# distributed-lab/linea-stark-prover

Measured on AMD Instinct MI355X. Metric: prove time (s) + trace-rows/sec, 3x3 perm AIR @2^19; NTT HBM GB/s vs roofline, higher is better.
Workload: dtype fr253 (BLS12-377 Fr, 8x u32 Montgomery limbs); 1 GPU; 3x3 permutation AIR, 2^19 rows (w=8, q=4 quotient chunks, log_blowup 3, 33 queries, Poseidon2-w3 Merkle, FRI); log_n=19, width=8, fri_queries=33, parallelism=single-gpu

## Files before the change

linea_stark_prover_amd/csrc/capi.cpp:

```cpp
#include <hip/hip_runtime.h>

#include <algorithm>
#include <cstdlib>
#include <cstring>
#include <memory>
#include <thread>

#include "comm.hpp"
#include "prove_internal.hpp"

using namespace lsp;

namespace {
thread_local std::string g_err;

#ifdef LSP_DEBUG_BOUNDS
std::string bounds_fault_report() {
    int n = 0;
    if (hipGetDeviceCount(&n) != hipSuccess || n == 0) return "";
    (void)hipDeviceSynchronize();
    static const struct {
        const char* tu;
        unsigned (*reader)();
    } tus[] = {{"k_ntt.hip", bounds_fault_k_ntt},         {"k_hash.hip", bounds_fault_k_hash},
// ... 1573 lines not shown
            });
        } else {
            const Fr* b = d + (size_t)na * height;
            const Fr* af = b + (size_t)t->ntables * t->nbc * height;
            const Fr* bf = af + height;
            witness_block(ctx, trace, height, trace_w, col0, w, mem, [&](Fr* out, size_t stride) {
                witness_lookup_device(ctx, d, na, b, t->ntables, t->nbc, af, bf, height, al, de, out, stride);
            });
        }
        ctx->sync();
    });
}

int lsp_raw_trace_free(lsp_raw_trace* t) {
    delete t;
    return LSP_OK;
}

int lsp_calibrate_poseidon2(lsp_ctx* ctx, double* mperm_per_s) {
    return guarded(ctx, [&] {
        LSP_REQUIRE(ctx && mperm_per_s, LSP_E_ARG, "null");
        std::lock_guard<std::mutex> g(ctx->mu);
        need_gpu(ctx);
        const uint32_t iters = 4;
        Fr* out = ctx->fbuf("calib", (size_t)256 * 256 * 32);
        LSP_HIP(launch_calib_perm(out, (size_t)256 * 256 * 4, 1, ctx->rc29_dev, ctx->p2.L, ctx->stream));
        StreamTimer timer;
        double best = 0;
        for (size_t per_cu : {2, 4, 8, 16, 32}) {
            const size_t nth = (size_t)256 * 256 * per_cu;
            const float ms = timer.ms(ctx->stream, [&] {
                LSP_HIP(launch_calib_perm(out, nth, iters, ctx->rc29_dev, ctx->p2.L, ctx->stream));
            });
            best = std::max(best, (double)nth * iters / (ms * 1e-3) / 1e6);
        }
        *mperm_per_s = best;
    });
}

int lsp_calibrate_intt(lsp_ctx* ctx, uint32_t log_h, size_t w, double* gelem_per_s) {
    return guarded(ctx, [&] {
        LSP_REQUIRE(ctx && gelem_per_s, LSP_E_ARG, "null argument");
        LSP_REQUIRE(log_h >= 1 && log_h <= 26 && w >= 1 && w <= 1024 && (w << log_h) <= ((size_t)1 << 28), LSP_E_ARG,
                    "bad inverse-NTT probe shape (at most 2^28 elements)");
        std::lock_guard<std::mutex> g(ctx->mu);
        need_gpu(ctx);
        *gelem_per_s = calibrate_intt(ctx, log_h, w, 5, nullptr);
        ctx->release("calib_intt_");
    });
}

int lsp_gen_permutation_trace(uint64_t seed, uint32_t log_n, uint32_t ncols, const lsp_fr* alpha,
                              const lsp_fr* delta, int small_values, lsp_fr* rows) {
    return guarded(nullptr, [&] {
        LSP_REQUIRE(alpha && delta && rows && ncols >= 1 && log_n >= 1 && log_n <= 30, LSP_E_ARG,
                    "bad trace arguments");
        const size_t n = (size_t)1 << log_n, w = 2 * (size_t)ncols + 2;
        SplitMix64 g{seed ^ 0x5452414345ull};
        std::vector<Fr> a((size_t)ncols * n);
// ... 44 lines not shown
```

linea_stark_prover_amd/csrc/host.cpp:

```cpp
#include "host.hpp"

#include <algorithm>
#include <array>
#include <chrono>
#include <cstdlib>
#include <cstring>

#if defined(__linux__)
#include <sched.h>
#endif

#include "comm.hpp"

namespace lsp {

Fr host_generator() { return fr_from_u64(22); }

Fr host_inv_cached(const Fr& a) {
    static std::mutex mu;
    static std::map<std::array<uint32_t, 8>, Fr> cache;
    std::array<uint32_t, 8> k;
    for (int i = 0; i < 8; ++i) k[i] = a.v[i];
    {
        std::lock_guard<std::mutex> g(mu);
// ... 372 lines not shown
}

}

lsp_ctx::~lsp_ctx() {
    delete comm;
    if (device == LSP_HOST_ONLY || !stream) return;
    (void)hipSetDevice(device);
    (void)hipStreamSynchronize(stream);
    if (side_stream) (void)hipStreamSynchronize(side_stream);
    for (auto& kv : pool)
        if (kv.second.p) (void)hipFree(kv.second.p);
    for (auto& kv : hpool)
        if (kv.second.p) (void)hipHostFree(kv.second.p);
    for (auto& kv : stage_ev) (void)hipEventDestroy(kv.second);
    for (hipEvent_t e : event_pool) (void)hipEventDestroy(e);
    for (auto& t : pending_timings) {
        (void)hipEventDestroy(std::get<1>(t));
        (void)hipEventDestroy(std::get<2>(t));
    }
    if (ev_near) (void)hipEventDestroy(ev_near);
    if (ev_top) (void)hipEventDestroy(ev_top);
    if (ev_warm) (void)hipEventDestroy(ev_warm);
    if (side_stream) {
        (void)hipStreamSynchronize(side_stream);
        (void)hipEventDestroy(ev_wide);
        (void)hipEventDestroy(ev_side);
        (void)hipStreamDestroy(side_stream);
    }
    if (rc_dev) (void)hipFree(rc_dev);
    if (rc29_dev) (void)hipFree(rc29_dev);
    (void)hipStreamDestroy(stream);
}

void* lsp_ctx::buf(const std::string& name, size_t bytes) {
    Buf& b = pool[name];
    if (b.cap < bytes) {
        if (b.p) {
            LSP_HIP(hipStreamSynchronize(stream));
            LSP_HIP(hipFree(b.p));
            b.p = nullptr;
            b.cap = 0;
        }
        if (bytes) {
            hipError_t e = hipMalloc(&b.p, bytes);
            if (e != hipSuccess) {
// ... 102 lines not shown
```

linea_stark_prover_amd/csrc/host.hpp:

```cpp
#pragma once
#include <hip/hip_runtime.h>

#include <algorithm>
#include <atomic>
#include <condition_variable>
#include <functional>
#include <map>
#include <memory>
#include <mutex>
#include <thread>
#include <tuple>
#include <stdexcept>
#include <string>
#include <utility>
#include <vector>

#include "../../include/lsp.h"
#include "air_walk.hpp"
#include "fr.hpp"
#include "kernels.hpp"
#include "poseidon2.hpp"
#include "poseidon2_host64.hpp"

namespace lsp {
// ... 382 lines not shown
    int device = 0;
    lsp::Comm* comm = nullptr;
    std::unique_ptr<lsp::HostPool> pool_;
    size_t host_tree_top = 1024;
    hipStream_t stream = nullptr;
    lsp::P2Host p2;
    lsp::Fr* rc_dev = nullptr;
    lsp::F29* rc29_dev = nullptr;
    uint32_t log_blowup = 3, log_final_poly_len = 0, num_queries = 33, pow_bits = 0;
    size_t lds_per_block = 64 * 1024;
    int32_t public_degree = 1;
    lsp::TranscriptCfg transcript;
    std::string err;
    std::mutex mu;
    struct Buf {
        void* p = nullptr;
        size_t cap = 0;
    };
    std::map<std::string, Buf> pool;
    std::map<std::string, Buf> hpool;
    std::map<std::string, hipEvent_t> stage_ev;
    hipEvent_t ev_near = nullptr, ev_top = nullptr;
    hipEvent_t ev_warm = nullptr;
    hipStream_t side_stream = nullptr;
    hipEvent_t ev_wide = nullptr, ev_side = nullptr;
    hipStream_t side();
    std::vector<hipEvent_t> event_pool;
    bool phase_timing = true;
    std::vector<std::string> phase_only;
    std::map<std::string, const lsp::Fr*> tables;
    const lsp::Fr* table(const std::string& key, size_t n, const std::function<void(lsp::Fr*)>& fill,
                         const char* scratch = nullptr);
    struct TopUpload {
        void* dst;
        const void* src;
        size_t bytes;
    };
    bool defer_top_uploads = false;
    std::vector<TopUpload> top_uploads;
    std::map<uint32_t, std::vector<lsp::Fr>> fold_tw;
    size_t fri_host_tail = 2048;
    std::vector<std::pair<std::string, double>> timings;
    std::vector<std::tuple<std::string, hipEvent_t, hipEvent_t>> pending_timings;
    std::vector<std::string> spans;

    void* buf(const std::string& name, size_t bytes);
// ... 14 lines not shown
```

linea_stark_prover_amd/csrc/k_hash.hip:

```cpp
#include <cstdlib>

#include "k_common.hpp"
#include "kernels.hpp"
#include "p2_launch.hpp"
#include "poseidon2_f29.hpp"
#include "poseidon2_row.hpp"

namespace lsp {

#ifndef LSP_P2_ROWS_WPE
#define LSP_P2_ROWS_WPE 1
#endif

namespace {
template <uint32_t D>
__global__ __launch_bounds__(256) void k_permute(Fr* __restrict__ st, size_t n, const F29* __restrict__ rc,
                                                 uint32_t rf, uint32_t rp) {
    __shared__ uint4 qt[3 * F29_QTAB_N];
    f29_qtab_init(qt);
    __syncthreads();
    const size_t i = gtid();
    if (i >= n) return;
    F29 s0 = f29_from_fr(st[3 * i]), s1 = f29_from_fr(st[3 * i + 1]), s2 = f29_from_fr(st[3 * i + 2]);
    permute3_any<D, 1>(s0, s1, s2, rc, rf, rp, qt);
// ... 192 lines not shown

hipError_t launch_merkle_level(const Fr* src, Fr* dst, size_t nout, const F29* rc, P2Layout L, hipStream_t st) {
    if (!nout) return hipSuccess;
    if (!L.gen_lin && nout <= row_max()) {
        if (L.sbox_degree == 17)
            hipLaunchKernelGGL(k_merkle_level_row<17>, dim3((unsigned)nout), dim3(64), 0, st, src, dst, nout, rc,
                               L.rounds_f, L.rounds_p);
        else
            hipLaunchKernelGGL(k_merkle_level_row<11>, dim3((unsigned)nout), dim3(64), 0, st, src, dst, nout, rc,
                               L.rounds_f, L.rounds_p);
        return hipGetLastError();
    }
    const int lanes = lanes_for(nout);
    unsigned blocks, bs;
    state_grid(nout, lanes, blocks, bs);
    p2_dispatch(L, lanes, [&](auto d, auto ln) {
        hipLaunchKernelGGL((k_merkle_level<decltype(d)::value, decltype(ln)::value>), dim3(blocks), dim3(bs), 0, st,
                           src, dst, nout, rc, L.rounds_f, L.rounds_p);
    });
    return hipGetLastError();
}

hipError_t launch_merkle_levels(Fr* layers, size_t nleaves, size_t stop_len, const F29* rc, P2Layout L,
                                size_t* off_out, size_t* len_out, hipStream_t st) {
    size_t off = 0, len = nleaves;
    while (len > stop_len && len > 1) {
        hipError_t e = launch_merkle_level(layers + off, layers + off + len, len / 2, rc, L, st);
        if (e != hipSuccess) return e;
        off += len;
        len /= 2;
    }
    *off_out = off;
    *len_out = len;
    return hipSuccess;
}

hipError_t launch_merkle_tree(Fr* layers, size_t nleaves, const F29* rc, P2Layout L, hipStream_t st) {
    size_t off = 0, len = nleaves;
    while (len > 128) {
        const size_t nout = len / 2;
        hipError_t e = launch_merkle_level(layers + off, layers + off + len, nout, rc, L, st);
        if (e != hipSuccess) return e;
        off += len;
        len /= 2;
    }
    if (len > 1) {
        p2_dispatch(L, [&](auto d) {
            hipLaunchKernelGGL(k_merkle_top<decltype(d)::value>, dim3(1), dim3(256), 0, st, layers, off, (uint32_t)len,
                               rc, L.rounds_f, L.rounds_p);
        });
// ... 9 lines not shown
```

linea_stark_prover_amd/csrc/kernels.hpp:

```cpp
#pragma once
#include <hip/hip_runtime.h>
#include <stddef.h>
#include <stdint.h>

#include "fr.hpp"
#include "fr29.hpp"
#include "ntt_plan.hpp"
#include "poseidon2.hpp"

namespace lsp {

constexpr uint32_t COLMAP_PLAIN = 0xffu;
struct ColMap {
    uint32_t logb = COLMAP_PLAIN;
    uint32_t stride = 0, c0 = 0, cstep = 1, valid = 0xffffffffu;
    uint32_t bw = 0;
    static ColMap plain(uint32_t w) {
        ColMap m;
        m.stride = w;
        m.valid = w;
        return m;
    }
    static ColMap blocked(uint32_t logb, uint32_t bw) {
        ColMap m;
// ... 28 lines not shown
                             Fr* tabs, hipStream_t st);
hipError_t launch_powers(const Fr* tab, uint32_t L1, size_t n, Fr* out, hipStream_t st);

struct MatList {
    const Fr* ptr[8];
    uint32_t width[8];
    uint32_t n;
};
inline MatList one_mat(const Fr* p, uint32_t w) {
    MatList m{};
    m.ptr[0] = p;
    m.width[0] = w;
    m.n = 1;
    return m;
}
hipError_t launch_rc_to_f29(const Fr* rc, F29* rc29, uint32_t n, hipStream_t st);
hipError_t launch_permute(Fr* states, size_t n, const F29* rc29, P2Layout L, hipStream_t st);
hipError_t launch_hash_rows(const MatList& m, size_t nrows, Fr* out, const F29* rc29, P2Layout L, hipStream_t st);
hipError_t launch_merkle_level(const Fr* src, Fr* dst, size_t nout, const F29* rc29, P2Layout L, hipStream_t st);
hipError_t launch_grind(const Fr pre[3], uint32_t wlane, uint64_t base, uint64_t count, uint32_t bits, bool mont,
                        const F29* rc29, P2Layout L, unsigned long long* best, hipStream_t st);
hipError_t launch_merkle_tree(Fr* layers, size_t nleaves, const F29* rc29, P2Layout L, hipStream_t st);
hipError_t launch_merkle_levels(Fr* layers, size_t nleaves, size_t stop_len, const F29* rc29, P2Layout L,
                                size_t* off_out, size_t* len_out, hipStream_t st);

hipError_t launch_merkle_inject(const Fr* src, const Fr* inj, Fr* dst, size_t nout, const F29* rc29, P2Layout L,
                                hipStream_t st);

struct FoldSpec {
    const Fr* v;
    Fr* vout;
    Fr half, half_beta;
    const Fr* tab;
    uint32_t L1, logm;
    uint64_t i0;
    const Fr* add;
};
hipError_t launch_fold_hash(const FoldSpec& f, size_t nleaves, Fr* out, const F29* rc29, P2Layout L, hipStream_t st);
hipError_t launch_fri_fold(const FoldSpec& f, size_t m, hipStream_t st);

size_t batch_inverse_scratch(size_t n);
hipError_t launch_batch_inverse(const Fr* in, Fr* out, size_t n, hipStream_t st, Fr* scratch,
                                const Fr* inv_total = nullptr);
hipError_t launch_calib_mul(Fr* out, size_t nthreads, uint32_t iters, hipStream_t st);
hipError_t launch_calib_perm(Fr* out, size_t nthreads, uint32_t iters, const F29* rc, P2Layout L, hipStream_t st);
hipError_t launch_gather(const uint64_t* ptrs, Fr* out, size_t n, hipStream_t st);
hipError_t launch_assemble_chunks(const Fr* stage, uint32_t logGq, size_t Sq, Fr* out, hipStream_t st);
// ... 125 lines not shown
```

linea_stark_prover_amd/csrc/merkle.cpp:

```cpp
#include <hip/hip_runtime.h>

#include <algorithm>
#include <atomic>
#include <chrono>
#include <cstdio>
#include <cstdlib>

#include "comm.hpp"
#include "host.hpp"
#include "prove_internal.hpp"

namespace lsp {

struct TopTimes {
    bool on = std::getenv("LSP_TIME_TOPS") != nullptr;
    double sync_us = 0, levels_us = 0, first_us = 0;
    size_t n = 0;
    struct Rec { size_t height; double since_prev, launch, near, spin, levels; };
    std::vector<Rec> recs;
    host_clock::time_point last_exit{};
    ~TopTimes() {
        if (on && n) {
            std::fprintf(stderr, "[tree tops] %zu trees: wait-for-GPU %.1f us, host levels %.1f us (first level %.1f us) per tree\n",
                         n, sync_us / n, levels_us / n, first_us / n);
            const size_t k = recs.size() < 16 ? 0 : recs.size() - 16;
            for (size_t i = k; i < recs.size(); ++i)
                std::fprintf(stderr, "[tree] height %9zu  since-prev %7.1f  launch %6.1f  near %8.1f  spin %7.1f  levels %6.1f us\n",
                             recs[i].height, recs[i].since_prev, recs[i].launch, recs[i].near, recs[i].spin, recs[i].levels);
        }
    }
};
static TopTimes g_top_times;
bool time_tops() { return g_top_times.on; }

static std::atomic<int> g_active_proofs{0};
ActiveProof::ActiveProof() { g_active_proofs.fetch_add(1, std::memory_order_relaxed); }
ActiveProof::~ActiveProof() { g_active_proofs.fetch_sub(1, std::memory_order_relaxed); }
constexpr size_t SHARED_HOST_TREE_TOP = 256;

static void host_compress_level(lsp_ctx* ctx, const Fr* in, Fr* out, size_t half) {
    HostPool& pool = ctx->host_pool();
    if (half <= pool.size())
        pool.parallel_for(half, [&](size_t i) { out[i] = ctx->p2.compress(in[2 * i], in[2 * i + 1]); });
    else {
        const size_t blk = half >= 16 * pool.size() ? 16 : 8;
        pool.parallel_for((half + blk - 1) / blk, [&](size_t b) {
            ctx->p2.compress_range(in, out, blk * b, std::min(half, blk * b + blk));
        });
    }
}

// ... 38 lines not shown
    }
    size_t P = 1;
    while (2 * P <= pool.size() && first / (2 * P) >= 16) P *= 2;
    const size_t per = first / P;
    const uint32_t sl = log2_exact(per);
    auto task = [&](size_t p) {
        if (pairs) leaf_part(p * per, per);
        for (uint32_t j = 1; j <= sl; ++j) level_part(j, p * (per >> j), per >> j);
    };
    if (P > 1)
        pool.parallel_for(P, task);
    else
        task(0);
    if (t_first) *t_first = std::chrono::steady_clock::now();
    for (uint32_t j = sl + 1; j <= nl; ++j) level_part(j, 0, first >> j);
    return end;
}

static std::string top_buf_name(lsp_ctx* ctx) {
    return ctx->defer_top_uploads ? "merkle_top" + std::to_string(ctx->top_uploads.size()) : std::string("merkle_top");
}

void flush_top_uploads(lsp_ctx* ctx) {
    for (const auto& u : ctx->top_uploads)
        LSP_HIP(hipMemcpyAsync(u.dst, u.src, u.bytes, hipMemcpyHostToDevice, ctx->stream));
    ctx->top_uploads.clear();
}

DeferTopUploads::DeferTopUploads(lsp_ctx* c) : ctx(c) {
    ctx->top_uploads.clear();
    ctx->defer_top_uploads = std::getenv("LSP_NO_DEFER_TOPS") == nullptr;
}
DeferTopUploads::~DeferTopUploads() {
    ctx->defer_top_uploads = false;
    ctx->top_uploads.clear();
}

static bool zerocopy_top() {
    static const bool on = [] {
        const char* e = std::getenv("LSP_TOP_ZEROCOPY");
        return !(e && *e == '0');
    }();
    return on;
}

constexpr size_t WIDE_LEVEL_STOP = (size_t)1 << 16;

static size_t top_warm_nodes(const lsp_ctx* ctx) {
    if (const char* e = std::getenv("LSP_TOP_WARM")) return (size_t)std::strtoull(e, nullptr, 10);
    static const bool shared_host = [] {
        const char* e = std::getenv("LOCAL_WORLD_SIZE");
        return e && std::strtol(e, nullptr, 10) > 1;
    }();
    if (shared_host || ctx->comm || g_active_proofs.load(std::memory_order_relaxed) > 1) return 0;
    return (size_t)1 << 20;
}
constexpr unsigned TOP_WARM_SPIN_US = 5000;

static void spin_until(hipEvent_t ev) {
    hipError_t q;
    while ((q = hipEventQuery(ev)) == hipErrorNotReady) {
#if defined(__x86_64__)
        __builtin_ia32_pause();
#endif
    }
    LSP_HIP(q);
}

size_t host_tree_top(const lsp_ctx* ctx) {
    size_t top = ctx->host_tree_top;
    if (g_active_proofs.load(std::memory_order_relaxed) > 1) top = std::min(top, SHARED_HOST_TREE_TOP);
    return env_size("LSP_HOST_TREE_TOP", top);
}

Fr commit_device(lsp_ctx* ctx, const MatList& m, size_t height, Fr* layers, size_t top, const FoldSpec* fold,
                 const std::function<void(hipEvent_t)>* side) {
    hipStream_t st = ctx->stream;
    using clk = host_clock;
    const auto tt0 = clk::now();
    auto t_launched = tt0, t_near = tt0;
    HostPool& pool = ctx->host_pool();
    size_t off = 0, len = height;
    if (fold && height <= top && height > 1) {
        LSP_HIP(launch_fri_fold(*fold, 2 * height, st));
        fold = nullptr;
    }
    const bool leaves_on_host = height <= top && m.n == 1 && height > 1;
    bool gpu_level_on_host = false;
    Fr* host;
    if (leaves_on_host) {
        const size_t w = m.width[0];
        host = (Fr*)ctx->hbuf(top_buf_name(ctx), (TreeLayout{height}.size() + height * w) * sizeof(Fr));
        Fr* rows = host + TreeLayout{height}.size();
        LSP_HIP(hipMemcpyAsync(rows, m.ptr[0], height * w * sizeof(Fr), hipMemcpyDeviceToHost, st));
        if (side) {
            LSP_HIP(hipEventRecord(ctx->ev_wide, st));
            (*side)(ctx->ev_wide);
        }
        LSP_HIP(hipStreamSynchronize(st));
        pool.parallel_for((height + 7) / 8, [&](size_t b) {
            ctx->p2.hash_range(rows, w, host, 8 * b, std::min(height, 8 * b + 8));
        });
    } else {
        if (fold)
            LSP_HIP(launch_fold_hash(*fold, height, layers, ctx->rc29_dev, ctx->p2.L, st));
        else
            LSP_HIP(launch_hash_rows(m, height, layers, ctx->rc29_dev, ctx->p2.L, st));
        if (top == 0) {
            LSP_HIP(launch_merkle_tree(layers, height, ctx->rc29_dev, ctx->p2.L, st));
            if (side) {
                LSP_HIP(hipEventRecord(ctx->ev_wide, st));
                (*side)(ctx->ev_wide);
            }
            return d2h_fr(ctx, layers + TreeLayout{height}.root());
        }
        if (!ctx->ev_near) {
            LSP_HIP(hipEventCreateWithFlags(&ctx->ev_near, hipEventDisableTiming));
            LSP_HIP(hipEventCreateWithFlags(&ctx->ev_top, hipEventDisableTiming));
            LSP_HIP(hipEventCreateWithFlags(&ctx->ev_warm, hipEventDisableTiming));
        }
        const size_t warm = top_warm_nodes(ctx);
        struct Stop {
            size_t nodes;
            hipEvent_t ev;
        } stops[2];
        int nstops = 0;
        if (warm) stops[nstops++] = {std::max(4 * top, warm), ctx->ev_warm};
        if (side) stops[nstops++] = {std::max(4 * top, WIDE_LEVEL_STOP), ctx->ev_wide};
        if (nstops == 2 && stops[1].nodes > stops[0].nodes) std::swap(stops[0], stops[1]);
        size_t off1 = 0, len1 = height;
        auto levels_to = [&](size_t stop, hipEvent_t ev = nullptr) {
            size_t o = 0, l = len1;
            LSP_HIP(launch_merkle_levels(layers + off1, len1, stop, ctx->rc29_dev, ctx->p2.L, &o, &l, st));
            if (ev) LSP_HIP(hipEventRecord(ev, st));
            off1 += o;
            len1 = l;
        };
        for (int k = 0; k < nstops; ++k) levels_to(stops[k].nodes, stops[k].ev);
        levels_to(4 * top, ctx->ev_near);
        if (zerocopy_top()) levels_to(2 * top);
        if (zerocopy_top() && len1 > top) {
            off = off1;
            len = len1 / 2;
            host = (Fr*)ctx->hbuf(top_buf_name(ctx) + "c", TreeLayout{len}.size() * sizeof(Fr), hipHostMallocCoherent);
            LSP_HIP(launch_merkle_level(layers + off, host, len, ctx->rc29_dev, ctx->p2.L, st));
            off += len1;
            gpu_level_on_host = true;
        } else {
            if (!zerocopy_top()) levels_to(top);
            off = off1;
            len = len1;
            host = (Fr*)ctx->hbuf(top_buf_name(ctx), TreeLayout{len}.size() * sizeof(Fr));
            LSP_HIP(hipMemcpyAsync(host, layers + off, len * sizeof(Fr), hipMemcpyDeviceToHost, st));
        }
        LSP_HIP(hipEventRecord(ctx->ev_top, st));
        if (side) (*side)(ctx->ev_wide);
        t_launched = clk::now();
        resolve_timings(ctx);
        if (warm) {
            LSP_HIP(hipEventSynchronize(ctx->ev_warm));
            pool.wake(TOP_WARM_SPIN_US);
            spin_until(ctx->ev_near);
            t_near = clk::now();
        } else {
            LSP_HIP(hipEventSynchronize(ctx->ev_near));
            t_near = clk::now();
            pool.wake();
        }
        spin_until(ctx->ev_top);
    }
    const auto tt1 = clk::now();
    auto tt2 = tt1;
    const size_t first = len;
    const size_t end = host_levels(ctx, host, first, &tt2);
    if (g_top_times.on) {
        const auto tt3 = clk::now();
        g_top_times.n++;
        g_top_times.sync_us += us(tt0, tt1);
        g_top_times.levels_us += us(tt1, tt3);
        g_top_times.first_us += us(tt1, tt2);
        g_top_times.recs.push_back({height, g_top_times.last_exit == clk::time_point{} ? 0.0 : us(g_top_times.last_exit, tt0),
                                    us(tt0, t_launched), us(t_launched, t_near), us(t_near, tt1), us(tt1, tt3)});
        g_top_times.last_exit = clk::now();
    }
    const size_t skip = leaves_on_host || gpu_level_on_host ? 0 : first;
    if (end > skip) {
        if (ctx->defer_top_uploads)
            ctx->top_uploads.push_back({layers + off + skip, host + skip, (end - skip) * sizeof(Fr)});
        else
            LSP_HIP(hipMemcpyAsync(layers + off + skip, host + skip, (end - skip) * sizeof(Fr), hipMemcpyHostToDevice, st));
    }
    return host[end - 1];
}

Fr shard_root(lsp_ctx* ctx, Comm& comm, const Fr& local, std::vector<std::vector<Fr>>& top, const char* tag) {
    if (comm.size == 1) {
        top.assign(1, std::vector<Fr>(1, local));
        return local;
    }
    top.assign(1, comm.allgather_fr(ctx, &local, 1, tag));
    while (top.back().size() > 1) {
        const std::vector<Fr>& lo = top.back();
        std::vector<Fr> up(lo.size() / 2);
        for (size_t i = 0; i < up.size(); ++i) up[i] = ctx->p2.compress(lo[2 * i], lo[2 * i + 1]);
        top.push_back(std::move(up));
// ... 6 lines not shown
```

linea_stark_prover_amd/csrc/merkle_mixed.cpp:

```cpp
#include <hip/hip_runtime.h>

#include <algorithm>

#include "host.hpp"
#include "prove_internal.hpp"

namespace lsp {

std::vector<HeightClass> height_classes(const size_t* widths, const size_t* heights, size_t nmats) {
    LSP_REQUIRE(widths && heights && nmats >= 1, LSP_E_ARG, "a batch needs at least one matrix");
    std::vector<size_t> order(nmats);
    for (size_t k = 0; k < nmats; ++k) {
        LSP_REQUIRE(widths[k] >= 1 && widths[k] <= ((size_t)1 << 20), LSP_E_ARG, "matrix width outside [1, 2^20]");
        LSP_REQUIRE(heights[k] <= ((size_t)1 << 40), LSP_E_SIZE, "matrix height beyond 2^40");
        log2_exact(heights[k]);
        LSP_REQUIRE(heights[k] * widths[k] <= ((size_t)1 << 48), LSP_E_SIZE, "matrix beyond 2^48 elements");
        order[k] = k;
    }
    std::stable_sort(order.begin(), order.end(), [&](size_t a, size_t b) { return heights[a] > heights[b]; });
    std::vector<HeightClass> cls;
    for (size_t k : order) {
        if (cls.empty() || cls.back().height != heights[k]) cls.push_back({heights[k], {}});
        LSP_REQUIRE(cls.back().idx.size() < 8, LSP_E_ARG, "more than 8 matrices of one height");
        cls.back().idx.push_back(k);
    }
    return cls;
}
// ... 14 lines not shown
        (void)hipGetLastError();
        throw LspError(LSP_E_OOM, std::string("hipMalloc of ") + what + " failed");
    }
    return d;
}

std::unique_ptr<lsp_tree> new_tree(lsp_ctx* ctx, size_t leaves, size_t nmats, const size_t* heights,
                                   const size_t* widths, const lsp_fr* const* src, int mem) {
    auto t = std::make_unique<lsp_tree>(ctx, leaves);
    t->widths.assign(widths, widths + nmats);
    t->heights.assign(heights, heights + nmats);
    for (size_t k = 0; k < nmats; ++k) {
        const size_t n = heights[k] * widths[k];
        t->mats.push_back(dev_alloc_fr(n, "a tree's matrix"));
        if (src)
            LSP_HIP(hipMemcpyAsync(t->mats[k], src[k], n * sizeof(Fr),
                                   mem == LSP_MEM_DEVICE ? hipMemcpyDeviceToDevice : hipMemcpyHostToDevice,
                                   ctx->stream));
    }
    t->layers = dev_alloc_fr(TreeLayout{leaves}.size(), "a tree's layers");
    return t;
}

Fr commit_mixed_device(lsp_ctx* ctx, const std::vector<HeightClass>& cls, const Fr* const* mats, const size_t* widths,
                       Fr* layers) {
    hipStream_t st = ctx->stream;
    const TreeLayout lay{cls[0].height};
    for (const HeightClass& c : cls) {
        MatList m{};
        m.n = (uint32_t)c.idx.size();
        for (uint32_t j = 0; j < m.n; ++j) {
            m.ptr[j] = mats[c.idx[j]];
            m.width[j] = (uint32_t)widths[c.idx[j]];
        }
        LSP_HIP(launch_hash_rows(m, c.height, layers + lay.offset_of_len(c.height), ctx->rc29_dev, ctx->p2.L, st));
    }
    size_t off = 0, len = lay.leaves, next = 1;
    while (len > 1) {
        if (next == cls.size()) {
            LSP_HIP(launch_merkle_tree(layers + off, len, ctx->rc29_dev, ctx->p2.L, st));
            break;
        }
        const size_t nout = len / 2;
        Fr* dst = layers + off + len;
        if (cls[next].height == nout) {
            LSP_HIP(launch_merkle_inject(layers + off, dst, dst, nout, ctx->rc29_dev, ctx->p2.L, st));
            ++next;
        } else
            LSP_HIP(launch_merkle_level(layers + off, dst, nout, ctx->rc29_dev, ctx->p2.L, st));
        off += len;
        len = nout;
    }
    return d2h_fr(ctx, layers + lay.root());
}

bool verify_mixed_host(const lsp_ctx* ctx, const Fr& root, const std::vector<HeightClass>& cls, const size_t* widths,
                       size_t nmats, size_t index, const lsp_fr* rows, const lsp_fr* path) {
    std::vector<size_t> at(nmats + 1, 0);
    for (size_t k = 0; k < nmats; ++k) at[k + 1] = at[k] + widths[k];
    auto class_hash = [&](const HeightClass& c) {
// ... 18 lines not shown
```

linea_stark_prover_amd/csrc/p2_launch.hpp:

```cpp
#pragma once
#include <cstdlib>
#include <type_traits>

#include "k_common.hpp"
#include "poseidon2.hpp"
#include "poseidon2_f29.hpp"

namespace lsp {

inline size_t p2_env_size(const char* name, size_t dflt) {
    const char* e = std::getenv(name);
    return e ? (size_t)std::strtoull(e, nullptr, 10) : dflt;
}
inline size_t coop_max() {
    static const size_t v = p2_env_size("LSP_COOP_MAX", 16384);
    return v;
}
inline size_t pair_max() {
    static const size_t v = p2_env_size("LSP_PAIR_MAX", 32768);
    return v;
}
inline unsigned coop_bs() {
    static const unsigned v = (unsigned)p2_env_size("LSP_COOP_BS", 0);
    return v;
}
inline int lanes_for(size_t n) { return n <= coop_max() ? 4 : (n <= pair_max() ? 2 : 1); }

inline void state_grid(size_t n, int lanes, unsigned& blocks, unsigned& bs) {
    bs = lanes == 4 ? (coop_bs() ? coop_bs() : (4 * n >= 65536 ? 256u : 64u)) : 256u;
    blocks = nblocks((size_t)lanes * n, bs);
}

template <class F>
inline void p2_dispatch(const P2Layout& L, F&& f) {
    if (L.gen_lin) {
        if (L.sbox_degree == 17)
            f(std::integral_constant<uint32_t, 17u | P2_GEN>{});
        else
            f(std::integral_constant<uint32_t, 11u | P2_GEN>{});
    } else if (L.sbox_degree == 17)
        f(std::integral_constant<uint32_t, 17u>{});
    else
        f(std::integral_constant<uint32_t, 11u>{});
}
template <class F>
inline void p2_dispatch(const P2Layout& L, int lanes, F&& f) {
    p2_dispatch(L, [&](auto d) {
        if (lanes == 4)
            f(d, std::integral_constant<int, 4>{});
        else if (lanes == 2)
            f(d, std::integral_constant<int, 2>{});
        else
// ... 6 lines not shown
```

linea_stark_prover_amd/csrc/prove_internal.hpp:

```cpp
#pragma once
#include <chrono>
#include <cstdlib>
#include <functional>
#include <string>
#include <vector>

#include "host.hpp"

namespace lsp {
struct Comm;
bool time_tops();
using host_clock = std::chrono::steady_clock;
inline double us(host_clock::time_point a, host_clock::time_point b) {
    return std::chrono::duration<double, std::micro>(b - a).count();
}
inline size_t env_size(const char* name, size_t dflt) {
    const char* e = std::getenv(name);
    return e ? (size_t)std::strtoull(e, nullptr, 10) : dflt;
}
const Fr* pow_table(lsp_ctx* ctx, const Fr& base, uint32_t bits, uint32_t& L1);
Fr d2h_fr(lsp_ctx* ctx, const Fr* d);
struct LdeRequest {
    const Fr* src = nullptr;
    bool coeffs = false;
// ... 43 lines not shown
};
template <class Sibling, class AfterLevel>
Fr merkle_path_root(const P2Host& p2, Fr cur, size_t index, uint32_t levels, Sibling&& sibling,
                    AfterLevel&& after_level) {
    for (uint32_t l = 0; l < levels; ++l) {
        const Fr sib = sibling(l);
        cur = after_level(l + 1, ((index >> l) & 1) ? p2.compress(sib, cur) : p2.compress(cur, sib));
    }
    return cur;
}
inline Fr no_injection(uint32_t, const Fr& cur) { return cur; }
std::unique_ptr<lsp_tree> new_tree(lsp_ctx* ctx, size_t leaves, size_t nmats, const size_t* heights,
                                   const size_t* widths, const lsp_fr* const* src, int mem);
struct ActiveProof {
    ActiveProof();
    ~ActiveProof();
};
struct DeferTopUploads {
    lsp_ctx* ctx;
    explicit DeferTopUploads(lsp_ctx* c);
    ~DeferTopUploads();
};
void flush_top_uploads(lsp_ctx* ctx);
size_t host_levels(lsp_ctx* ctx, Fr* host, size_t first, host_clock::time_point* t_first = nullptr,
                   const Fr* pairs = nullptr);
Fr shard_root(lsp_ctx* ctx, Comm& comm, const Fr& local, std::vector<std::vector<Fr>>& top, const char* tag);
void lde_device(lsp_ctx* ctx, const Fr* d_in, size_t h, size_t w, uint32_t added_bits, const Fr* shifts_host,
                Fr* d_out);
void coset_dft_device(lsp_ctx* ctx, const Fr* d_coef, size_t h, size_t w, const Fr& shift, Fr* d_out);
void coset_idft_device(lsp_ctx* ctx, const Fr* d_evals, size_t h, size_t w, const Fr& shift, Fr* d_out);
void resolve_timings(lsp_ctx* ctx);
size_t host_tree_top(const lsp_ctx* ctx);
Fr commit_device(lsp_ctx* ctx, const MatList& m, size_t height, Fr* layers, size_t top, const FoldSpec* fold = nullptr,
                 const std::function<void(hipEvent_t)>* side = nullptr);
struct HeightClass {
    size_t height;
    std::vector<size_t> idx;
};
std::vector<HeightClass> height_classes(const size_t* widths, const size_t* heights, size_t nmats);
Fr commit_mixed_device(lsp_ctx* ctx, const std::vector<HeightClass>& cls, const Fr* const* mats, const size_t* widths,
                       Fr* layers);
bool verify_mixed_host(const lsp_ctx* ctx, const Fr& root, const std::vector<HeightClass>& cls, const size_t* widths,
                       size_t nmats, size_t index, const lsp_fr* rows, const lsp_fr* path);
uint64_t grind_device(lsp_ctx* ctx, Challenger& ch, uint32_t bits);
struct FriRound {
    const Fr* vec;
// ... 128 lines not shown
```

Baseline: 8.653 million trace-rows/s.

## Offload tail slice of large Merkle leaf hashing to host thread pool

For large commit trees (at least 2^21 leaves, single proof, zero-copy top), the last 1/32 to 1/128 of leaf rows is copied to the host on the side stream. There the CPU pool hashes and compresses that slice into the join level while the GPU hashes the remaining prefix. The slice size is picked from one-time calibrated GPU and host Poseidon2 permutation rates, and the host-computed layers are uploaded back into the device tree. The intent is to shave GPU hashing time by using idle CPU cores, at the cost of extra D2H/H2D traffic, a first-call calibration, and more synchronisation. Separately, the 4-lane cooperative block size now switches to 256 threads at a lower element count.

Result: faster. 8.740 million trace-rows/s, median of 6 (+1.0%).

```diff
diff --git a/linea_stark_prover_amd/csrc/capi.cpp b/linea_stark_prover_amd/csrc/capi.cpp
--- a/linea_stark_prover_amd/csrc/capi.cpp
+++ b/linea_stark_prover_amd/csrc/capi.cpp
@@ -1619,19 +1619,7 @@
         LSP_REQUIRE(ctx && mperm_per_s, LSP_E_ARG, "null");
         std::lock_guard<std::mutex> g(ctx->mu);
         need_gpu(ctx);
-        const uint32_t iters = 4;
-        Fr* out = ctx->fbuf("calib", (size_t)256 * 256 * 32);
-        LSP_HIP(launch_calib_perm(out, (size_t)256 * 256 * 4, 1, ctx->rc29_dev, ctx->p2.L, ctx->stream));
-        StreamTimer timer;
-        double best = 0;
-        for (size_t per_cu : {2, 4, 8, 16, 32}) {
-            const size_t nth = (size_t)256 * 256 * per_cu;
-            const float ms = timer.ms(ctx->stream, [&] {
-                LSP_HIP(launch_calib_perm(out, nth, iters, ctx->rc29_dev, ctx->p2.L, ctx->stream));
-            });
-            best = std::max(best, (double)nth * iters / (ms * 1e-3) / 1e6);
-        }
-        *mperm_per_s = best;
+        *mperm_per_s = calibrate_poseidon2(ctx);
     });
 }
 
diff --git a/linea_stark_prover_amd/csrc/host.cpp b/linea_stark_prover_amd/csrc/host.cpp
--- a/linea_stark_prover_amd/csrc/host.cpp
+++ b/linea_stark_prover_amd/csrc/host.cpp
@@ -418,6 +418,9 @@
     if (ev_near) (void)hipEventDestroy(ev_near);
     if (ev_top) (void)hipEventDestroy(ev_top);
     if (ev_warm) (void)hipEventDestroy(ev_warm);
+    if (ev_slice_in) (void)hipEventDestroy(ev_slice_in);
+    if (ev_slice) (void)hipEventDestroy(ev_slice);
+    if (ev_slice_up) (void)hipEventDestroy(ev_slice_up);
     if (side_stream) {
         (void)hipStreamSynchronize(side_stream);
         (void)hipEventDestroy(ev_wide);
diff --git a/linea_stark_prover_amd/csrc/host.hpp b/linea_stark_prover_amd/csrc/host.hpp
--- a/linea_stark_prover_amd/csrc/host.hpp
+++ b/linea_stark_prover_amd/csrc/host.hpp
@@ -428,6 +428,10 @@
     std::map<std::string, hipEvent_t> stage_ev;
     hipEvent_t ev_near = nullptr, ev_top = nullptr;
     hipEvent_t ev_warm = nullptr;
+    hipEvent_t ev_slice_in = nullptr, ev_slice = nullptr;
+    double slice_host_perm_s = 0, slice_gpu_perm_s = 0;
+    hipEvent_t ev_slice_up = nullptr;
+    bool slice_uploads_pending = false;
     hipStream_t side_stream = nullptr;
     hipEvent_t ev_wide = nullptr, ev_side = nullptr;
     hipStream_t side();
diff --git a/linea_stark_prover_amd/csrc/host_slice.hpp b/linea_stark_prover_amd/csrc/host_slice.hpp
--- /dev/null
+++ b/linea_stark_prover_amd/csrc/host_slice.hpp
@@ -0,0 +1,52 @@
+#pragma once
+#include <cstddef>
+#include <cstdint>
+
+namespace lsp {
+
+constexpr size_t HOST_SLICE_MIN_LEAVES = (size_t)1 << 21;
+constexpr double HOST_SLICE_MARGIN = 0.85;
+constexpr uint32_t HOST_SLICE_LOG_FRAC_FIRST = 5, HOST_SLICE_LOG_FRAC_LAST = 7;
+
+struct HostSliceIn {
+    size_t leaves = 0;
+    size_t perms_per_leaf = 1;
+    size_t join = 0;
+    double host_perm_s = 0;
+    double gpu_perm_s = 0;
+    bool shared = false;
+    int forced = -1;
+};
+
+struct HostSlice {
+    uint32_t log_frac = 0;
+    explicit operator bool() const { return log_frac != 0; }
+    size_t slice(size_t len) const { return log_frac ? len >> log_frac : 0; }
+    size_t prefix(size_t len) const { return len - slice(len); }
+};
+
+inline double slice_perms(size_t leaves, size_t perms_per_leaf, size_t roots) {
+    return (double)leaves * (double)perms_per_leaf + (double)(leaves - roots);
+}
+
+inline bool host_slice_fits(const HostSliceIn& in, uint32_t log_frac) {
+    if (log_frac == 0 || log_frac >= 8 * sizeof(size_t)) return false;
+    if (in.join == 0 || (in.join & (in.join - 1)) || in.leaves <= in.join || (in.leaves & (in.leaves - 1))) return false;
+    return (in.join >> log_frac) >= 1;
+}
+
+inline HostSlice plan_host_slice(const HostSliceIn& in) {
+    if (in.forced == 0) return {};
+    if (in.forced > 0) return host_slice_fits(in, (uint32_t)in.forced) ? HostSlice{(uint32_t)in.forced} : HostSlice{};
+    if (in.shared || in.leaves < HOST_SLICE_MIN_LEAVES || !(in.host_perm_s > 0) || !(in.gpu_perm_s > 0)) return {};
+    for (uint32_t lf = HOST_SLICE_LOG_FRAC_FIRST; lf <= HOST_SLICE_LOG_FRAC_LAST; ++lf) {
+        if (!host_slice_fits(in, lf)) break;
+        const HostSlice s{lf};
+        const double host_s = slice_perms(s.slice(in.leaves), in.perms_per_leaf, s.slice(in.join)) / in.host_perm_s;
+        const double gpu_s = slice_perms(s.prefix(in.leaves), in.perms_per_leaf, s.prefix(in.join)) / in.gpu_perm_s;
+        if (host_s <= HOST_SLICE_MARGIN * gpu_s) return s;
+    }
+    return {};
+}
+
+}
diff --git a/linea_stark_prover_amd/csrc/k_hash.hip b/linea_stark_prover_amd/csrc/k_hash.hip
--- a/linea_stark_prover_amd/csrc/k_hash.hip
+++ b/linea_stark_prover_amd/csrc/k_hash.hip
@@ -238,10 +238,11 @@
 }
 
 hipError_t launch_merkle_levels(Fr* layers, size_t nleaves, size_t stop_len, const F29* rc, P2Layout L,
-                                size_t* off_out, size_t* len_out, hipStream_t st) {
+                                size_t* off_out, size_t* len_out, hipStream_t st, uint32_t skip_log_frac) {
     size_t off = 0, len = nleaves;
     while (len > stop_len && len > 1) {
-        hipError_t e = launch_merkle_level(layers + off, layers + off + len, len / 2, rc, L, st);
+        const size_t nout = len / 2, skip = skip_log_frac ? nout >> skip_log_frac : 0;
+        hipError_t e = launch_merkle_level(layers + off, layers + off + len, nout - skip, rc, L, st);
         if (e != hipSuccess) return e;
         off += len;
         len /= 2;
diff --git a/linea_stark_prover_amd/csrc/kernels.hpp b/linea_stark_prover_amd/csrc/kernels.hpp
--- a/linea_stark_prover_amd/csrc/kernels.hpp
+++ b/linea_stark_prover_amd/csrc/kernels.hpp
@@ -74,7 +74,7 @@
                         const F29* rc29, P2Layout L, unsigned long long* best, hipStream_t st);
 hipError_t launch_merkle_tree(Fr* layers, size_t nleaves, const F29* rc29, P2Layout L, hipStream_t st);
 hipError_t launch_merkle_levels(Fr* layers, size_t nleaves, size_t stop_len, const F29* rc29, P2Layout L,
-                                size_t* off_out, size_t* len_out, hipStream_t st);
+                                size_t* off_out, size_t* len_out, hipStream_t st, uint32_t skip_log_frac = 0);
 
 hipError_t launch_merkle_inject(const Fr* src, const Fr* inj, Fr* dst, size_t nout, const F29* rc29, P2Layout L,
                                 hipStream_t st);
diff --git a/linea_stark_prover_amd/csrc/merkle.cpp b/linea_stark_prover_amd/csrc/merkle.cpp
--- a/linea_stark_prover_amd/csrc/merkle.cpp
+++ b/linea_stark_prover_amd/csrc/merkle.cpp
@@ -8,6 +8,7 @@
 
 #include "comm.hpp"
 #include "host.hpp"
+#include "host_slice.hpp"
 #include "prove_internal.hpp"
 
 namespace lsp {
@@ -16,7 +17,7 @@
     bool on = std::getenv("LSP_TIME_TOPS") != nullptr;
     double sync_us = 0, levels_us = 0, first_us = 0;
     size_t n = 0;
-    struct Rec { size_t height; double since_prev, launch, near, spin, levels; };
+    struct Rec { size_t height; double since_prev, launch, near, spin, levels, slice; };
     std::vector<Rec> recs;
     host_clock::time_point last_exit{};
     ~TopTimes() {
@@ -25,8 +26,8 @@
                          n, sync_us / n, levels_us / n, first_us / n);
             const size_t k = recs.size() < 16 ? 0 : recs.size() - 16;
             for (size_t i = k; i < recs.size(); ++i)
-                std::fprintf(stderr, "[tree] height %9zu  since-prev %7.1f  launch %6.1f  near %8.1f  spin %7.1f  levels %6.1f us\n",
-                             recs[i].height, recs[i].since_prev, recs[i].launch, recs[i].near, recs[i].spin, recs[i].levels);
+                std::fprintf(stderr, "[tree] height %9zu  since-prev %7.1f  launch %6.1f  near %8.1f  spin %7.1f  levels %6.1f  host slice %8.1f us\n",
+                             recs[i].height, recs[i].since_prev, recs[i].launch, recs[i].near, recs[i].spin, recs[i].levels, recs[i].slice);
         }
     }
 };
@@ -111,6 +112,10 @@
 }
 
 void flush_top_uploads(lsp_ctx* ctx) {
+    if (ctx->slice_uploads_pending) {
+        LSP_HIP(hipStreamWaitEvent(ctx->stream, ctx->ev_slice_up, 0));
+        ctx->slice_uploads_pending = false;
+    }
     for (const auto& u : ctx->top_uploads)
         LSP_HIP(hipMemcpyAsync(u.dst, u.src, u.bytes, hipMemcpyHostToDevice, ctx->stream));
     ctx->top_uploads.clear();
@@ -122,6 +127,7 @@
 }
 DeferTopUploads::~DeferTopUploads() {
     ctx->defer_top_uploads = false;
+    ctx->slice_uploads_pending = false;
     ctx->top_uploads.clear();
 }
 
@@ -135,13 +141,16 @@
 
 constexpr size_t WIDE_LEVEL_STOP = (size_t)1 << 16;
 
-static size_t top_warm_nodes(const lsp_ctx* ctx) {
-    if (const char* e = std::getenv("LSP_TOP_WARM")) return (size_t)std::strtoull(e, nullptr, 10);
-    static const bool shared_host = [] {
+static bool shared_host() {
+    static const bool v = [] {
         const char* e = std::getenv("LOCAL_WORLD_SIZE");
         return e && std::strtol(e, nullptr, 10) > 1;
     }();
-    if (shared_host || ctx->comm || g_active_proofs.load(std::memory_order_relaxed) > 1) return 0;
+    return v;
+}
+static size_t top_warm_nodes(const lsp_ctx* ctx) {
+    if (const char* e = std::getenv("LSP_TOP_WARM")) return (size_t)std::strtoull(e, nullptr, 10);
+    if (shared_host() || ctx->comm || g_active_proofs.load(std::memory_order_relaxed) > 1) return 0;
     return (size_t)1 << 20;
 }
 constexpr unsigned TOP_WARM_SPIN_US = 5000;
@@ -160,6 +169,159 @@
     size_t top = ctx->host_tree_top;
     if (g_active_proofs.load(std::memory_order_relaxed) > 1) top = std::min(top, SHARED_HOST_TREE_TOP);
     return env_size("LSP_HOST_TREE_TOP", top);
+}
+
+double calibrate_poseidon2(lsp_ctx* ctx) {
+    const uint32_t iters = 4;
+    Fr* out = ctx->fbuf("calib", (size_t)256 * 256 * 32);
+    LSP_HIP(launch_calib_perm(out, (size_t)256 * 256 * 4, 1, ctx->rc29_dev, ctx->p2.L, ctx->stream));
+    StreamTimer timer;
+    double best = 0;
+    for (size_t per_cu : {2, 4, 8, 16, 32}) {
+        const size_t nth = (size_t)256 * 256 * per_cu;
+        const float ms = timer.ms(ctx->stream, [&] {
+            LSP_HIP(launch_calib_perm(out, nth, iters, ctx->rc29_dev, ctx->p2.L, ctx->stream));
+        });
+        best = std::max(best, (double)nth * iters / (ms * 1e-3) / 1e6);
+    }
+    return best;
+}
+
+static double host_pool_perm_rate(lsp_ctx* ctx) {
+    HostPool& pool = ctx->host_pool();
+    const size_t per = 256, w = 8, tasks = 8 * (size_t)pool.size();
+    std::vector<Fr> rows(per * w * tasks), lay(2 * per * tasks);
+    for (size_t i = 0; i < rows.size(); ++i) rows[i] = fr_from_u64(i + 1);
+    double best = 0;
+    for (int rep = 0; rep < 4; ++rep) {
+        const auto t0 = host_clock::now();
+        pool.parallel_for(tasks, [&](size_t t) {
+            Fr* l = lay.data() + 2 * per * t;
+            ctx->p2.hash_range(rows.data() + per * w * t, w, l, 0, per);
+            for (size_t n = per / 2; n >= 1; l += 2 * n, n /= 2) ctx->p2.compress_range(l, l + 2 * n, 0, n);
+        });
+        const double s = us(t0, host_clock::now()) * 1e-6;
+        if (rep) best = std::max(best, (double)(tasks * (per * w / 2 + per - 1)) / s);
+    }
+    return best;
+}
+
+static HostSlice plan_slice(lsp_ctx* ctx, const MatList& m, size_t height, size_t top) {
+    HostSliceIn in;
+    const char* e = std::getenv("LSP_HOST_SLICE");
+    in.forced = e ? std::max(-1, (int)std::strtol(e, nullptr, 10)) : -1;
+    if (in.forced == 0 || !zerocopy_top() || top == 0 || height < 2 * top) return {};
+    in.leaves = height;
+    in.join = top;
+    size_t w = 0;
+    for (uint32_t k = 0; k < m.n; ++k) w += m.width[k];
+    in.perms_per_leaf = (w + 1) / 2;
+    in.shared = shared_host() || ctx->comm || g_active_proofs.load(std::memory_order_relaxed) != 1;
+    if (in.forced < 0) {
+        if (in.shared || height < HOST_SLICE_MIN_LEAVES) return {};
+        if (!(ctx->slice_host_perm_s > 0)) {
+            ctx->slice_gpu_perm_s = calibrate_poseidon2(ctx) * 1e6;
+            ctx->slice_host_perm_s = host_pool_perm_rate(ctx);
+            if (g_top_times.on)
+                std::fprintf(stderr, "[host slice] rates: host pool %.1f, GPU %.1f M permutations/s\n",
+                             ctx->slice_host_perm_s * 1e-6, ctx->slice_gpu_perm_s * 1e-6);
+        }
+        in.host_perm_s = ctx->slice_host_perm_s;
+        in.gpu_perm_s = ctx->slice_gpu_perm_s;
+    }
+    return plan_host_slice(in);
+}
+
+struct SliceBuf {
+    HostSlice hs;
+    size_t S = 0, J = 0, W = 0;
+    uint32_t nj = 0;
+    Fr* buf = nullptr;
+    Fr* rows() const { return buf + TreeLayout{S}.offset(nj); }
+};
+
+hipStream_t slice_stream_begin(lsp_ctx* ctx) {
+    if (!ctx->ev_slice) {
+        LSP_HIP(hipEventCreateWithFlags(&ctx->ev_slice_in, hipEventDisableTiming));
+        LSP_HIP(hipEventCreateWithFlags(&ctx->ev_slice, hipEventDisableTiming));
+        LSP_HIP(hipEventCreateWithFlags(&ctx->ev_slice_up, hipEventDisableTiming));
+    }
+    hipStream_t sd = ctx->side();
+    LSP_HIP(hipEventRecord(ctx->ev_slice_in, ctx->stream));
+    LSP_HIP(hipStreamWaitEvent(sd, ctx->ev_slice_in, 0));
+    return sd;
+}
+void slice_stream_end(lsp_ctx* ctx) { LSP_HIP(hipEventRecord(ctx->ev_slice, ctx->side())); }
+
+void host_hash_rows(const P2Host& p2, const Fr* const* rows, const size_t* width, size_t n, Fr* out, size_t i0,
+                    size_t i1) {
+    if (n == 1) {
+        p2.hash_range(rows[0], width[0], out, i0, i1);
+        return;
+    }
+    size_t W = 0;
+    for (size_t k = 0; k < n; ++k) W += width[k];
+    std::vector<Fr> cat((i1 - i0) * W);
+    for (size_t k = 0, c0 = 0; k < n; c0 += width[k++])
+        for (size_t i = i0; i < i1; ++i)
+            std::copy(rows[k] + i * width[k], rows[k] + (i + 1) * width[k], &cat[(i - i0) * W + c0]);
+    p2.hash_range(cat.data(), W, out + i0, 0, i1 - i0);
+}
+
+static SliceBuf slice_download(lsp_ctx* ctx, const MatList& m, size_t height, size_t top, HostSlice hs,
+                               const std::string& name) {
+    SliceBuf b;
+    b.hs = hs;
+    b.S = hs.slice(height);
+    b.J = hs.slice(top);
+    b.nj = log2_exact(b.S / b.J);
+    for (uint32_t k = 0; k < m.n; ++k) b.W += m.width[k];
+    b.buf = (Fr*)ctx->hbuf(name, (TreeLayout{b.S}.offset(b.nj) + b.S * b.W) * sizeof(Fr));
+    hipStream_t sd = slice_stream_begin(ctx);
+    Fr* dst = b.rows();
+    for (uint32_t k = 0; k < m.n; ++k) {
+        const size_t w = m.width[k];
+        LSP_HIP(hipMemcpyAsync(dst, m.ptr[k] + (height - b.S) * w, b.S * w * sizeof(Fr), hipMemcpyDeviceToHost, sd));
+        dst += b.S * w;
+    }
+    slice_stream_end(ctx);
+    return b;
+}
+
+static void slice_hash(lsp_ctx* ctx, const MatList& m, size_t height, const SliceBuf& b, Fr* join, Fr* layers) {
+    LSP_HIP(hipEventSynchronize(ctx->ev_slice));
+    HostPool& pool = ctx->host_pool();
+    const TreeLayout sl{b.S};
+    auto level = [&](uint32_t j) { return j == b.nj ? join : b.buf + sl.offset(j); };
+    const size_t per = std::min<size_t>(b.S / b.J, 256);
+    const uint32_t lp = log2_exact(per);
+    const Fr* rows[8];
+    size_t width[8];
+    for (uint32_t k = 0; k < m.n; ++k) {
+        width[k] = m.width[k];
+        rows[k] = k ? rows[k - 1] + b.S * width[k - 1] : b.rows();
+    }
+    pool.parallel_for(b.S / per, [&](size_t t) {
+        const size_t i0 = t * per;
+        host_hash_rows(ctx->p2, rows, width, m.n, level(0), i0, i0 + per);
+        for (uint32_t j = 1; j <= lp; ++j) ctx->p2.compress_range(level(j - 1), level(j), i0 >> j, (i0 + per) >> j);
+    });
+    if (lp < b.nj)
+        pool.parallel_for(b.J, [&](size_t p) {
+            for (uint32_t j = lp + 1; j <= b.nj; ++j) {
+                const size_t c = (b.S >> j) / b.J;
+                ctx->p2.compress_range(level(j - 1), level(j), p * c, (p + 1) * c);
+            }
+        });
+    const TreeLayout lay{height};
+    hipStream_t up = ctx->defer_top_uploads ? ctx->side() : ctx->stream;
+    for (uint32_t j = 0; j < b.nj; ++j)
+        LSP_HIP(hipMemcpyAsync(layers + lay.offset(j) + b.hs.prefix(lay.len(j)), level(j), (b.S >> j) * sizeof(Fr),
+                               hipMemcpyHostToDevice, up));
+    if (ctx->defer_top_uploads) {
+        LSP_HIP(hipEventRecord(ctx->ev_slice_up, up));
+        ctx->slice_uploads_pending = true;
+    }
 }
 
 Fr commit_device(lsp_ctx* ctx, const MatList& m, size_t height, Fr* layers, size_t top, const FoldSpec* fold,
@@ -177,9 +339,11 @@
     const bool leaves_on_host = height <= top && m.n == 1 && height > 1;
     bool gpu_level_on_host = false;
     Fr* host;
+    const std::string tbuf = top_buf_name(ctx);
+    double slice_us = 0;
     if (leaves_on_host) {
         const size_t w = m.width[0];
-        host = (Fr*)ctx->hbuf(top_buf_name(ctx), (TreeLayout{height}.size() + height * w) * sizeof(Fr));
+        host = (Fr*)ctx->hbuf(tbuf, (TreeLayout{height}.size() + height * w) * sizeof(Fr));
         Fr* rows = host + TreeLayout{height}.size();
         LSP_HIP(hipMemcpyAsync(rows, m.ptr[0], height * w * sizeof(Fr), hipMemcpyDeviceToHost, st));
         if (side) {
@@ -191,10 +355,13 @@
             ctx->p2.hash_range(rows, w, host, 8 * b, std::min(height, 8 * b + 8));
         });
     } else {
+        const HostSlice hs = fold ? HostSlice{} : plan_slice(ctx, m, height, top);
+        SliceBuf sb;
+        if (hs) sb = slice_download(ctx, m, height, top, hs, tbuf + "s");
         if (fold)
             LSP_HIP(launch_fold_hash(*fold, height, layers, ctx->rc29_dev, ctx->p2.L, st));
         else
-            LSP_HIP(launch_hash_rows(m, height, layers, ctx->rc29_dev, ctx->p2.L, st));
+            LSP_HIP(launch_hash_rows(m, hs.prefix(height), layers, ctx->rc29_dev, ctx->p2.L, st));
         if (top == 0) {
             LSP_HIP(launch_merkle_tree(layers, height, ctx->rc29_dev, ctx->p2.L, st));
             if (side) {
@@ -220,7 +387,7 @@
         size_t off1 = 0, len1 = height;
         auto levels_to = [&](size_t stop, hipEvent_t ev = nullptr) {
             size_t o = 0, l = len1;
-            LSP_HIP(launch_merkle_levels(layers + off1, len1, stop, ctx->rc29_dev, ctx->p2.L, &o, &l, st));
+            LSP_HIP(launch_merkle_levels(layers + off1, len1, stop, ctx->rc29_dev, ctx->p2.L, &o, &l, st, hs.log_frac));
             if (ev) LSP_HIP(hipEventRecord(ev, st));
             off1 += o;
             len1 = l;
@@ -231,21 +398,27 @@
         if (zerocopy_top() && len1 > top) {
             off = off1;
             len = len1 / 2;
-            host = (Fr*)ctx->hbuf(top_buf_name(ctx) + "c", TreeLayout{len}.size() * sizeof(Fr), hipHostMallocCoherent);
-            LSP_HIP(launch_merkle_level(layers + off, host, len, ctx->rc29_dev, ctx->p2.L, st));
+            host = (Fr*)ctx->hbuf(tbuf + "c", TreeLayout{len}.size() * sizeof(Fr), hipHostMallocCoherent);
+            LSP_HIP(launch_merkle_level(layers + off, host, hs.prefix(len), ctx->rc29_dev, ctx->p2.L, st));
             off += len1;
             gpu_level_on_host = true;
         } else {
             if (!zerocopy_top()) levels_to(top);
             off = off1;
             len = len1;
-            host = (Fr*)ctx->hbuf(top_buf_name(ctx), TreeLayout{len}.size() * sizeof(Fr));
+            LSP_REQUIRE(!hs, LSP_E_STATE, "a host slice without the coherent tree top");
+            host = (Fr*)ctx->hbuf(tbuf, TreeLayout{len}.size() * sizeof(Fr));
             LSP_HIP(hipMemcpyAsync(host, layers + off, len * sizeof(Fr), hipMemcpyDeviceToHost, st));
         }
         LSP_HIP(hipEventRecord(ctx->ev_top, st));
         if (side) (*side)(ctx->ev_wide);
         t_launched = clk::now();
         resolve_timings(ctx);
+        if (hs) {
+            const auto ts0 = clk::now();
+            slice_hash(ctx, m, height, sb, host + hs.prefix(len), layers);
+            slice_us = us(ts0, clk::now());
+        }
         if (warm) {
             LSP_HIP(hipEventSynchronize(ctx->ev_warm));
             pool.wake(TOP_WARM_SPIN_US);
@@ -269,7 +442,7 @@
         g_top_times.levels_us += us(tt1, tt3);
         g_top_times.first_us += us(tt1, tt2);
         g_top_times.recs.push_back({height, g_top_times.last_exit == clk::time_point{} ? 0.0 : us(g_top_times.last_exit, tt0),
-                                    us(tt0, t_launched), us(t_launched, t_near), us(t_near, tt1), us(tt1, tt3)});
+                                    us(tt0, t_launched), us(t_launched, t_near), us(t_near, tt1), us(tt1, tt3), slice_us});
         g_top_times.last_exit = clk::now();
     }
     const size_t skip = leaves_on_host || gpu_level_on_host ? 0 : first;
diff --git a/linea_stark_prover_amd/csrc/merkle_mixed.cpp b/linea_stark_prover_amd/csrc/merkle_mixed.cpp
--- a/linea_stark_prover_amd/csrc/merkle_mixed.cpp
+++ b/linea_stark_prover_amd/csrc/merkle_mixed.cpp
@@ -1,8 +1,11 @@
 #include <hip/hip_runtime.h>
 
 #include <algorithm>
+#include <cstdlib>
+#include <functional>
 
 #include "host.hpp"
+#include "host_slice.hpp"
 #include "prove_internal.hpp"
 
 namespace lsp {
@@ -63,10 +66,99 @@
     return t;
 }
 
+static HostSlice mixed_slice(size_t leaves) {
+    HostSliceIn in;
+    const char* e = std::getenv("LSP_HOST_SLICE");
+    in.forced = e ? (int)std::strtol(e, nullptr, 10) : 0;
+    if (in.forced <= 0 || in.forced >= 40) return {};
+    in.leaves = leaves;
+    in.join = (size_t)1 << in.forced;
+    return plan_host_slice(in);
+}
+
+namespace {
+struct MixedSlice {
+    HostSlice hs;
+    size_t S = 0;
+    Fr* buf = nullptr;
+    std::vector<const Fr*> rows;
+};
+}
+
+static MixedSlice mixed_slice_download(lsp_ctx* ctx, const std::vector<HeightClass>& cls, const Fr* const* mats,
+                                       const size_t* widths, HostSlice hs) {
+    MixedSlice s;
+    s.hs = hs;
+    s.S = hs.slice(cls[0].height);
+    size_t elems = 0, nmats = 0;
+    for (const HeightClass& c : cls)
+        for (size_t k : c.idx) {
+            elems += hs.slice(c.height) * widths[k];
+            nmats = std::max(nmats, k + 1);
+        }
+    s.rows.assign(nmats, nullptr);
+    s.buf = (Fr*)ctx->hbuf("merkle_mixed_slice", (TreeLayout{s.S}.size() + elems) * sizeof(Fr));
+    hipStream_t sd = slice_stream_begin(ctx);
+    Fr* dst = s.buf + TreeLayout{s.S}.size();
+    for (const HeightClass& c : cls) {
+        const size_t n = hs.slice(c.height);
+        for (size_t k : c.idx) {
+            if (!n) continue;
+            LSP_HIP(hipMemcpyAsync(dst, mats[k] + (c.height - n) * widths[k], n * widths[k] * sizeof(Fr),
+                                   hipMemcpyDeviceToHost, sd));
+            s.rows[k] = dst;
+            dst += n * widths[k];
+        }
+    }
+    slice_stream_end(ctx);
+    return s;
+}
+
+static void mixed_slice_hash(lsp_ctx* ctx, const std::vector<HeightClass>& cls, const size_t* widths,
+                             const MixedSlice& s, Fr* layers) {
+    LSP_HIP(hipEventSynchronize(ctx->ev_slice));
+    HostPool& pool = ctx->host_pool();
+    const TreeLayout lay{cls[0].height}, sl{s.S};
+    auto chunks = [&](size_t n, const std::function<void(size_t, size_t)>& f) {
+        pool.parallel_for((n + 63) / 64, [&](size_t b) { f(64 * b, std::min(n, 64 * b + 64)); });
+    };
+    auto class_digests = [&](const HeightClass& c, Fr* out, size_t n) {
+        const Fr* rows[8];
+        size_t w[8];
+        for (size_t j = 0; j < c.idx.size(); ++j) {
+            rows[j] = s.rows[c.idx[j]];
+            w[j] = widths[c.idx[j]];
+        }
+        chunks(n, [&](size_t i0, size_t i1) { host_hash_rows(ctx->p2, rows, w, c.idx.size(), out, i0, i1); });
+    };
+    class_digests(cls[0], s.buf, s.S);
+    std::vector<Fr> inj;
+    size_t next = 1;
+    for (uint32_t j = 1; j <= sl.levels(); ++j) {
+        const Fr* in = s.buf + sl.offset(j - 1);
+        Fr* out = s.buf + sl.offset(j);
+        const size_t nout = sl.len(j);
+        chunks(nout, [&](size_t i0, size_t i1) { ctx->p2.compress_range(in, out, i0, i1); });
+        if (next < cls.size() && cls[next].height == lay.len(j)) {
+            inj.resize(nout);
+            class_digests(cls[next++], inj.data(), nout);
+            chunks(nout, [&](size_t i0, size_t i1) {
+                for (size_t i = i0; i < i1; ++i) out[i] = ctx->p2.compress(out[i], inj[i]);
+            });
+        }
+    }
+    for (uint32_t j = 0; j <= sl.levels(); ++j)
+        LSP_HIP(hipMemcpyAsync(layers + lay.offset(j) + s.hs.prefix(lay.len(j)), s.buf + sl.offset(j),
+                               sl.len(j) * sizeof(Fr), hipMemcpyHostToDevice, ctx->stream));
+}
+
 Fr commit_mixed_device(lsp_ctx* ctx, const std::vector<HeightClass>& cls, const Fr* const* mats, const size_t* widths,
                        Fr* layers) {
     hipStream_t st = ctx->stream;
     const TreeLayout lay{cls[0].height};
+    const HostSlice hs = mixed_slice(lay.leaves);
+    MixedSlice sl;
+    if (hs) sl = mixed_slice_download(ctx, cls, mats, widths, hs);
     for (const HeightClass& c : cls) {
         MatList m{};
         m.n = (uint32_t)c.idx.size();
@@ -74,9 +166,24 @@
             m.ptr[j] = mats[c.idx[j]];
             m.width[j] = (uint32_t)widths[c.idx[j]];
         }
-        LSP_HIP(launch_hash_rows(m, c.height, layers + lay.offset_of_len(c.height), ctx->rc29_dev, ctx->p2.L, st));
+        LSP_HIP(launch_hash_rows(m, hs.prefix(c.height), layers + lay.offset_of_len(c.height), ctx->rc29_dev,
+                                 ctx->p2.L, st));
     }
     size_t off = 0, len = lay.leaves, next = 1;
+    if (hs) {
+        while (hs.slice(len / 2) >= 1) {
+            const size_t nout = len / 2;
+            Fr* dst = layers + off + len;
+            if (next < cls.size() && cls[next].height == nout) {
+                LSP_HIP(launch_merkle_inject(layers + off, dst, dst, hs.prefix(nout), ctx->rc29_dev, ctx->p2.L, st));
+                ++next;
+            } else
+                LSP_HIP(launch_merkle_level(layers + off, dst, hs.prefix(nout), ctx->rc29_dev, ctx->p2.L, st));
+            off += len;
+            len = nout;
+        }
+        mixed_slice_hash(ctx, cls, widths, sl, layers);
+    }
     while (len > 1) {
         if (next == cls.size()) {
             LSP_HIP(launch_merkle_tree(layers + off, len, ctx->rc29_dev, ctx->p2.L, st));
diff --git a/linea_stark_prover_amd/csrc/p2_launch.hpp b/linea_stark_prover_amd/csrc/p2_launch.hpp
--- a/linea_stark_prover_amd/csrc/p2_launch.hpp
+++ b/linea_stark_prover_amd/csrc/p2_launch.hpp
@@ -27,7 +27,7 @@
 inline int lanes_for(size_t n) { return n <= coop_max() ? 4 : (n <= pair_max() ? 2 : 1); }
 
 inline void state_grid(size_t n, int lanes, unsigned& blocks, unsigned& bs) {
-    bs = lanes == 4 ? (coop_bs() ? coop_bs() : (4 * n >= 65536 ? 256u : 64u)) : 256u;
+    bs = lanes == 4 ? (coop_bs() ? coop_bs() : (n > 8192 ? 256u : 64u)) : 256u;
     blocks = nblocks((size_t)lanes * n, bs);
 }
 
diff --git a/linea_stark_prover_amd/csrc/prove_internal.hpp b/linea_stark_prover_amd/csrc/prove_internal.hpp
--- a/linea_stark_prover_amd/csrc/prove_internal.hpp
+++ b/linea_stark_prover_amd/csrc/prove_internal.hpp
@@ -89,6 +89,11 @@
     ~DeferTopUploads();
 };
 void flush_top_uploads(lsp_ctx* ctx);
+double calibrate_poseidon2(lsp_ctx* ctx);
+hipStream_t slice_stream_begin(lsp_ctx* ctx);
+void slice_stream_end(lsp_ctx* ctx);
+void host_hash_rows(const P2Host& p2, const Fr* const* rows, const size_t* width, size_t n, Fr* out, size_t i0,
+                    size_t i1);
 size_t host_levels(lsp_ctx* ctx, Fr* host, size_t first, host_clock::time_point* t_first = nullptr,
                    const Fr* pairs = nullptr);
 Fr shard_root(lsp_ctx* ctx, Comm& comm, const Fr& local, std::vector<std::vector<Fr>>& top, const char* tag);
```
